# shresthasagar/quantized_spectrum_cartography

Measured on AMD Instinct MI355X. Metric: MLE grad-steps/sec + SLF NMSE, 512x512x256 R=8, higher is better.
Workload: dtype f32; 1 GPU; c3: 512x512 grid, K=256, R=8, one-bit probit, f=0.1, free-S alternating Adam (C-step, S-step); K=256, R=8, parallelism=single, world_size=1, hipgraph=True, nnz_per_gpu=6711192, entry_bytes=2

## Files before the change

### include/qsc.h

```cpp
#ifndef QSC_H_
#define QSC_H_

#include <stddef.h>
#include <stdint.h>

#ifdef __cplusplus
extern "C" {
#endif

#define QSC_API __attribute__((visibility("default")))

#define QSC_OK 0
#define QSC_EINVAL 100000
#define QSC_EUNSUPPORTED 100001
#define QSC_MAX_BOUNDS 256
#define QSC_MAX_R 16
#define QSC_UNOBSERVED 0xFF

typedef struct qsc_model {
  int32_t nbounds;
  int32_t log_model;
  double sigma;
  double offset;
  float bounds[QSC_MAX_BOUNDS];
  int32_t loss;
  int32_t reserved_;
} qsc_model;
#define QSC_LOSS_PROBIT 0
#define QSC_LOSS_SQUARED 1
#define QSC_LOSS_LOGIT 2

typedef struct qsc_adam {
  double lr;
  double beta1;
  double beta2;
  double eps;
  int32_t project_nonneg;
  int32_t pad_;
} qsc_adam;

#define QSC_PEND_C 1
#define QSC_PEND_SNLL 2
#define QSC_PEND_SUPD 4
typedef struct qsc_state {
  int32_t step_c;
  int32_t step_s;
  int32_t iter;
  int32_t pending;
  float normsq_s;
  float normsq_c;
  float nll_c;
  float nll_s;
  float normsq_s_prev;
  int32_t fused_fault;
  uint64_t fin_ticket;
  float reserved[4];
} qsc_state;

#define QSC_SLICE 32
#define QSC_ENTRY_TAIL 256
typedef struct qsc_obs_desc {
  int32_t K;
  int32_t P;
  int32_t Pp;
  int32_t PT;
  int32_t ntiles;
  int32_t nks;
  int32_t wide;
  int32_t nbins;
  int64_t nnz;
  int64_t s_entries;
  int64_t c_entries;
  int32_t rowfmt;
  int32_t reserved_;
} qsc_obs_desc;

QSC_API int qsc_version(void);
QSC_API int qsc_rank_pad(int32_t R);
QSC_API const char* qsc_error_string(int code);
QSC_API int qsc_device_check(int dev);

QSC_API int qsc_quantize(const float* X, const float* noise, int64_t n, const qsc_model* m,
                         int64_t* Y, void* stream);
QSC_API int qsc_bin_codes(const float* x, int64_t n, const qsc_model* m, int64_t* Y,
                          void* stream);
QSC_API int qsc_prob_probit(const int64_t* Y, const float* Xhat, int64_t n, const qsc_model* m,
                            float* P, void* stream);
QSC_API int qsc_prob_probit_bwd(const int64_t* Y, const float* Xhat, const float* gP, int64_t n,
                                const qsc_model* m, float* gX, void* stream);
QSC_API int qsc_f_probit(const float* y, int64_t n, double sigma, float* out, void* stream);
QSC_API int qsc_f_logit(const float* y, int64_t n, double scale, float* out, void* stream);
QSC_API int qsc_prob_logit(const int64_t* Y, const float* Xhat, int64_t n, const qsc_model* m,
                           float* P, void* stream);
QSC_API int qsc_prob_logit_bwd(const int64_t* Y, const float* Xhat, const float* gP, int64_t n,
                               const qsc_model* m, float* gX, void* stream);
QSC_API int qsc_obs_from_ordinal(const int64_t* Y, int64_t n, const qsc_model* m, float* out,
                                 void* stream);
QSC_API int qsc_pack_codes(const int64_t* Y, const float* Wx, int64_t n, int32_t nbins,
                           uint8_t* codes, int32_t* bad, void* stream);

QSC_API int qsc_reconstruct(const float* S, const float* C, int32_t R, int32_t P, int32_t K,
                            float* T, void* stream);
QSC_API size_t qsc_reconstruct_bwd_workspace_bytes(int32_t R, int32_t P, int32_t K);
QSC_API int qsc_reconstruct_bwd(const float* gT, const float* S, const float* C, int32_t R,
                                int32_t P, int32_t K, float* dS, float* dC, void* ws,
                                size_t ws_bytes, void* stream);

QSC_API size_t qsc_reduce_workspace_bytes(int64_t n);
QSC_API int qsc_diff_sumsq(const float* a, const float* b, int64_t n, int32_t use_log,
                           double offset, double* out2, void* ws, size_t ws_bytes, void* stream);
QSC_API int qsc_map_diff_sumsq(const float* S, const float* C, const float* Ttrue, int32_t R,
                               int32_t P, int32_t K, int32_t use_log, double offset,
                               double* out2, void* ws, size_t ws_bytes, void* stream);
QSC_API int qsc_map_nmse_track(const float* S_pos, const int32_t* iperm, int32_t RP,
                               const float* C, const float* Ttrue, int32_t R, int32_t P,
                               int32_t K, int32_t use_log, double offset, const qsc_state* st,
                               int32_t every, double* hist, int32_t cap, void* ws,
                               size_t ws_bytes, void* stream);
QSC_API int qsc_sumsq(const float* x, int64_t n, float* out, void* ws, size_t ws_bytes,
                      void* stream);

QSC_API int qsc_obs_count(const uint8_t* codes, int32_t K, int32_t P, int32_t* cnt, void* stream);
QSC_API size_t qsc_obs_order_workspace_bytes(int32_t P);
QSC_API int qsc_obs_order(const int32_t* cnt, int32_t P, int32_t Pp, int32_t* perm, void* ws,
                          size_t ws_bytes, void* stream);
QSC_API size_t qsc_obs_layout_workspace_bytes(int32_t K, int32_t P, int32_t PT);
QSC_API int qsc_obs_layout(const uint8_t* codes, int32_t K, int32_t P, int32_t PT, int32_t nbins,
                           const int32_t* perm, const int32_t* cnt, int32_t* s_width,
                           int64_t* s_off, int32_t* c_width, int64_t* c_off, int32_t* c_kmap,
                           void* ws, size_t ws_bytes, qsc_obs_desc* desc, void* stream);
QSC_API int qsc_obs_signed_rows_ok(const qsc_obs_desc* desc, int32_t R, const qsc_model* m);
QSC_API int qsc_obs_fill(const uint8_t* codes, const qsc_obs_desc* desc, const int32_t* perm,
                         const int32_t* s_width, const int64_t* s_off, const int32_t* c_width,
                         const int64_t* c_off, const int32_t* c_kmap, void* s_entries,
                         void* c_entries, void* stream);
QSC_API size_t qsc_obs_schedule_workspace_bytes(const qsc_obs_desc* desc);
QSC_API int qsc_obs_schedule(const qsc_obs_desc* desc, const int32_t* s_width,
                             const int64_t* s_off, const int32_t* c_width, const int64_t* c_off,
                             void* s_entries, void* c_entries, void* ws, size_t ws_bytes,
                             void* stream);
QSC_API int qsc_sched_lists_host(const uint32_t* in, uint32_t* out, int32_t W, int32_t rowfmt,
                                 int32_t rows, int32_t wide);
QSC_API int qsc_perm_gather(const float* nat, const int32_t* perm, int32_t R, int32_t P,
                            int32_t Pp, float* pos, void* stream);
QSC_API int qsc_perm_scatter(const float* pos, const int32_t* perm, int32_t R, int32_t P,
                             int32_t Pp, float* nat, void* stream);

QSC_API size_t qsc_pass_workspace_bytes(const qsc_obs_desc* d, int32_t R);
QSC_API int qsc_state_init(qsc_state* st, const float* S, int32_t R, int32_t Pp, void* ws,
                           size_t ws_bytes, void* stream);
QSC_API int qsc_spass(const qsc_obs_desc* d, const void* s_entries, const int32_t* s_width,
                      const int64_t* s_off, const qsc_model* m, int32_t R, float* S,
                      const float* C, int32_t mode, float* dS, float* mS, float* vS,
                      const qsc_adam* adam, float lambda_s, qsc_state* st, void* ws,
                      size_t ws_bytes, void* stream);
QSC_API int qsc_spass_kslab(const qsc_obs_desc* d, const void* s_entries, const int32_t* s_width,
                            const int64_t* s_off, const qsc_model* m, int32_t R, float* S,
                            const float* C, float* dS_rs, int32_t chunk_slices, int32_t nranks,
                            qsc_state* st, void* ws, size_t ws_bytes, void* stream);
QSC_API int qsc_cpass(const qsc_obs_desc* d, const void* c_entries, const int32_t* c_width,
                      const int64_t* c_off, const int32_t* c_kmap, const qsc_model* m, int32_t R,
                      const float* S, const float* C, void* ws, size_t ws_bytes, void* stream);
QSC_API int qsc_scpass_supported(const qsc_obs_desc* d, int32_t R);
QSC_API int qsc_scpass(const qsc_obs_desc* d, const void* s_entries, const int32_t* s_width,
                       const int64_t* s_off, const void* c_entries, const int32_t* c_width,
                       const int64_t* c_off, const int32_t* c_kmap, const qsc_model* m,
                       int32_t R, float* S,
                       const float* C, float* mS, float* vS, const qsc_adam* adam,
                       float lambda_s, qsc_state* st, void* ws, size_t ws_bytes, void* stream);
QSC_API int qsc_cfinish(const qsc_obs_desc* d, int32_t R, float* C, int32_t mode, float* dC,
                        float* mC, float* vC, const qsc_adam* adam, float lambda_c,
                        const float* normsq_c_ext, qsc_state* st, float* hist,
                        int32_t hist_cap, void* ws, size_t ws_bytes, void* stream);
QSC_API int qsc_cupdate(int32_t R, int32_t K, float* C, float* mC, float* vC, const float* g,
                        const qsc_adam* adam, float lambda_c, const float* normsq_s_ext,
                        qsc_state* st, void* stream);
QSC_API int qsc_state_flush(const qsc_obs_desc* d, int32_t R, qsc_state* st, float* hist,
                            int32_t hist_cap, void* ws, size_t ws_bytes, void* stream);
QSC_API int qsc_supdate(const qsc_obs_desc* d, int32_t R, float* S, float* mS, float* vS,
                        const float* g, const qsc_adam* adam, float lambda_s, qsc_state* st,
                        void* ws, size_t ws_bytes, void* stream);
QSC_API int qsc_supdate_slices(const qsc_obs_desc* d, int32_t R, int32_t s0, int32_t s1,
                               float* S, float* mS, float* vS, const float* g_own,
                               const qsc_adam* adam, float lambda_s, qsc_state* st, void* ws,
                               size_t ws_bytes, void* stream);
QSC_API int qsc_slice_nsq(const qsc_obs_desc* d, int32_t R, const float* S, void* ws,
                          size_t ws_bytes, void* stream);
QSC_API int qsc_cpass_nsq(const qsc_obs_desc* d, const void* c_entries, const int32_t* c_width,
                          const int64_t* c_off, const int32_t* c_kmap, const qsc_model* m,
                          int32_t R, const float* S, const float* C, void* ws, size_t ws_bytes,
                          void* stream);
QSC_API int64_t qsc_pass_cnsq_offset(const qsc_obs_desc* d, int32_t R);
QSC_API int qsc_sumsq_small(const float* x, int32_t n, float* out, void* stream);
QSC_API int qsc_adam_flat(float* p, float* m, float* v, const float* g, int64_t n,
                          const qsc_adam* adam, const qsc_state* st, void* stream);
#define QSC_SMOOTH_QUAD 0
#define QSC_SMOOTH_HUBER 1
QSC_API size_t qsc_smooth_workspace_bytes(int32_t Pp);
QSC_API int qsc_smooth_neighbors(const int32_t* perm, int32_t P, int32_t Pp, int32_t I, int32_t J,
                                 int32_t* nbr, void* ws, size_t ws_bytes, void* stream);
QSC_API int qsc_smooth_grad(const float* S, const int32_t* nbr, int32_t R, int32_t Pp,
                            int32_t kind, float delta, float weight, float* dS, float* pen,
                            float* pen_hist, int32_t hist_cap, void* ws, size_t ws_bytes,
                            void* stream);

#define QSC_INFO_EXPECTED 0
#define QSC_INFO_OBSERVED 1
QSC_API int qsc_sinfo(const qsc_obs_desc* d, const void* s_entries, const int32_t* s_width,
                      const int64_t* s_off, const qsc_model* m, int32_t R, const float* S,
                      const float* C, int32_t kind, float* J, void* stream);
QSC_API int qsc_info_std(const float* J, const int32_t* perm, int32_t R, int32_t P, int32_t Pp,
                         const float* C, int32_t K, float ridge, float* std_S, float* std_T,
                         int32_t* nbad, void* stream);
QSC_API int qsc_entry_info(const int64_t* Y, const float* T, int64_t n, const qsc_model* m,
                           int32_t kind, float* H, void* stream);

#define QSC_DESIGN_D 0
#define QSC_DESIGN_A 1
#define QSC_DESIGN_V 2
QSC_API int qsc_sgain(const float* S, const float* C, const float* J, const int32_t* perm,
                      const float* w, const float* G, const qsc_model* m, int32_t R, int32_t K,
                      int32_t P, int32_t Pp, int32_t criterion, float ridge, float* gain,
                      int32_t* n_first, int32_t* n_bad, void* stream);

#define QSC_CHECK_UNTESTABLE 1
#define QSC_CHECK_INVALID 2
#define QSC_CHECK_SATURATED 4
QSC_API int qsc_scheck(const qsc_obs_desc* d, const void* s_entries, const int32_t* s_width,
                       const int64_t* s_off, const int32_t* perm, const qsc_model* m, int32_t R,
                       const float* S, const float* C, int32_t fitted, float ridge, float* stat,
                       int32_t* count, int32_t* flags, void* stream);
QSC_API int qsc_entry_check(const int64_t* Y, const float* T, int64_t n, const qsc_model* m,
                            float* out, void* stream);

QSC_API size_t qsc_sfit_workspace_bytes(const qsc_obs_desc* d, int32_t R);
QSC_API int qsc_sfit(const qsc_obs_desc* d, const void* s_entries, const int32_t* s_width,
                     const int64_t* s_off, const int32_t* perm, const qsc_model* m, int32_t R,
                     const float* C, const float* S_init, int32_t kind, float ridge, float mu0,
                     float tol, int32_t max_steps, int32_t project, float* S_out, float* f_out,
                     int32_t* steps, int32_t* n_unconverged, int32_t* n_unidentified, void* ws,
                     size_t ws_bytes, void* stream);

QSC_API size_t qsc_sfit_smooth_workspace_bytes(const qsc_obs_desc* d, int32_t R);
QSC_API int qsc_sfit_smooth(const qsc_obs_desc* d, const void* s_entries, const int32_t* s_width,
                            const int64_t* s_off, const int32_t* perm, const int32_t* nbr,
                            int32_t I, int32_t J, int32_t color, const qsc_model* m, int32_t R,
                            const float* C, float* S, int32_t kind, float ridge, float mu0,
                            float tol, int32_t inner_steps, int32_t project, int32_t smooth_kind,
                            float delta, float weight, float* f_out, float* nll_out,
                            int32_t* steps, int32_t* n_moved, int32_t* n_unconverged,
                            int32_t* n_unidentified, void* ws, size_t ws_bytes, void* stream);

QSC_API size_t qsc_cfit_workspace_bytes(const qsc_obs_desc* d, int32_t R);
QSC_API int32_t qsc_cfit_groups(const qsc_obs_desc* d, int32_t R);
QSC_API int64_t qsc_cfit_active_offset(void);
QSC_API int qsc_cfit_begin(const qsc_obs_desc* d, const void* c_entries, const int32_t* c_width,
                           const int64_t* c_off, const int32_t* c_kmap, const qsc_model* m,
                           int32_t R, const float* S, const float* C_init, int32_t kind,
                           float ridge, float mu0, float tol, int32_t max_steps, int32_t project,
                           void* ws, size_t ws_bytes, void* stream);
QSC_API int qsc_cfit_iterate(const qsc_obs_desc* d, const void* c_entries, const int32_t* c_width,
                             const int64_t* c_off, const int32_t* c_kmap, const qsc_model* m,
                             int32_t R, const float* S, int32_t kind, void* ws, size_t ws_bytes,
                             void* stream);
QSC_API int qsc_cfit_finish(const qsc_obs_desc* d, const qsc_model* m, int32_t R, float* C_out,
                            double* f_out, int32_t* steps, float* std_C, int32_t* n_unconverged,
                            int32_t* n_unidentified, void* ws, size_t ws_bytes, void* stream);

QSC_API int qsc_debug_status(int32_t clear);
QSC_API int qsc_selftest_erf(const float* x, int32_t n, float* out, void* stream);

QSC_API size_t qsc_gram_workspace_bytes(int32_t R, int32_t P, int32_t K);
QSC_API int qsc_gram(const float* S, const float* w, int32_t R, int32_t P, float* G, void* ws,
                     size_t ws_bytes, void* stream);
QSC_API int qsc_gram_rhs(const float* S, const float* T, const float* w, int32_t R, int32_t P,
                         int32_t K, float* B, void* ws, size_t ws_bytes, void* stream);
QSC_API int qsc_chol_solve(const float* G, const float* B, int32_t R, int32_t K, float lambda,
                           float* X, void* stream);

QSC_API size_t qsc_syrk_workspace_bytes(int32_t K, int32_t P);
QSC_API int qsc_syrk(const float* T, const float* w, int32_t K, int32_t P, float* G, void* ws,
                     size_t ws_bytes, void* stream);
QSC_API size_t qsc_spa_workspace_bytes(int32_t K, int32_t P, int32_t R);
QSC_API int qsc_spa(const float* T, const float* w, int32_t K, int32_t P, int32_t R,
                    int32_t* sel, int32_t* count, float* C, float* S, float* G_out, void* ws,
                    size_t ws_bytes, void* stream);
QSC_API int qsc_nnls(const float* G, const float* B, int32_t R, int32_t K, float lambda,
                     float* X, void* stream);

QSC_API size_t qsc_map_compose_workspace_bytes(int32_t R, int32_t I, int32_t J);
QSC_API int qsc_map_compose(const float* shadow, const float* loc, const float* alpha, int32_t R,
                            int32_t I, int32_t J, float res, float d0, int32_t db, float* S,
                            float* norms, void* ws, size_t ws_bytes, void* stream);

QSC_API int qsc_obs_readings_count(const int32_t* k, const int32_t* p, const void* code,
                                   int32_t code_bytes, int64_t n, int32_t K, int32_t P,
                                   int32_t nbins, int32_t* cnt, int32_t* bad, void* stream);
QSC_API size_t qsc_obs_readings_packed_bytes(int64_t n, int32_t K, int32_t P, int32_t PT);
QSC_API size_t qsc_obs_readings_workspace_bytes(int64_t n, int32_t K, int32_t P, int32_t PT);
QSC_API int qsc_obs_readings_layout(const int32_t* k, const int32_t* p, const void* code,
                                    int32_t code_bytes, int64_t n, int32_t K, int32_t P,
                                    int32_t PT, int32_t nbins, const int32_t* perm,
                                    const int32_t* cnt, int32_t* s_width, int64_t* s_off,
                                    int32_t* c_width, int64_t* c_off, int32_t* c_kmap,
                                    void* packed, size_t packed_bytes, void* ws, size_t ws_bytes,
                                    qsc_obs_desc* desc, int32_t* max_repeat, void* stream);
QSC_API int qsc_obs_readings_fill(const void* packed, size_t packed_bytes, int64_t n,
                                  const qsc_obs_desc* desc, const int32_t* s_width,
                                  const int64_t* s_off, const int32_t* c_width,
                                  const int64_t* c_off, const int32_t* c_kmap, void* s_entries,
                                  void* c_entries, void* stream);

#define QSC_QFIT_SCALE 1
#define QSC_QFIT_SHIFT 2
#define QSC_QFIT_UNCONVERGED 1
#define QSC_QFIT_UNIDENTIFIED 2
QSC_API size_t qsc_qfit_workspace_bytes(const qsc_obs_desc* d, int32_t R);
QSC_API int64_t qsc_qfit_active_offset(void);
QSC_API int qsc_qfit_begin(const qsc_obs_desc* d, const void* s_entries, const int32_t* s_width,
                           const int64_t* s_off, const qsc_model* m, int32_t R, const float* S,
                           const float* C, int32_t kind, int32_t fit_mask, double prior_scale,
                           double prior_shift, double tau0, double beta0, float mu0, float tol,
                           int32_t max_steps, void* ws, size_t ws_bytes, void* stream);
QSC_API int qsc_qfit_iterate(const qsc_obs_desc* d, const void* s_entries, const int32_t* s_width,
                             const int64_t* s_off, const qsc_model* m, int32_t R, const float* S,
                             const float* C, int32_t kind, void* ws, size_t ws_bytes,
                             void* stream);
QSC_API int qsc_qfit_finish(const qsc_obs_desc* d, const qsc_model* m, int32_t R,
                            double* theta_out, double* f_out, double* cov_out, double* gh_out,
                            int32_t* steps, int32_t* flags, void* ws, size_t ws_bytes,
                            void* stream);
QSC_API int qsc_entry_calib(const int64_t* Y, const float* T, int64_t n, const qsc_model* m,
                            double tau, double beta, int32_t kind, double* out, void* stream);

#ifdef __cplusplus
}
#endif
#endif
```

### quantized_spectrum_cartography_amd/csrc/qsc_pass_finish.hip

```cpp
#define QSC_PASS_NO_STAMPS
#include "qsc_pass_host.cuh"

namespace {

struct Canon {
  float nll_s, nsq_s, nll_c;
};

__device__ __forceinline__ float canon_part(const float* __restrict__ x, int n, int tid, int nb) {
  float a = 0.0f;
  if (!x) return a;
  for (int i0 = tid; i0 < n; i0 += 8 * nb) {
    float v[8];
#pragma unroll
    for (int j = 0; j < 8; ++j) v[j] = x[min(i0 + j * nb, n - 1)];
#pragma unroll
    for (int j = 0; j < 8; ++j)
      if (i0 + j * nb < n) a += v[j];
  }
  return a;
}

__device__ Canon canon_totals(const float* __restrict__ nll_s, const float* __restrict__ nsq_s,
                              const float* __restrict__ nll_c, int nslices, int nc, float* sh) {
  const int nb = blockDim.x, tid = threadIdx.x, nw = nb >> 6;
  float a = canon_part(nll_s, nslices, tid, nb);
  float b = canon_part(nsq_s, nslices, tid, nb);
  float c = canon_part(nll_c, nc, tid, nb);
  a = wave_sum(a);
  b = wave_sum(b);
  c = wave_sum(c);
  if ((tid & 63) == 0) {
    sh[tid >> 6] = a;
    sh[nw + (tid >> 6)] = b;
    sh[2 * nw + (tid >> 6)] = c;
  }
  __syncthreads();
  Canon r{0.0f, 0.0f, 0.0f};
  if (tid == 0)
    for (int w = 0; w < nw; ++w) {
      r.nll_s += sh[w];
      r.nsq_s += sh[nw + w];
      r.nll_c += sh[2 * nw + w];
    }
  return r;
}

__device__ void settle_s(qsc_state* __restrict__ st, const float* __restrict__ part_nll_s,
                         const float* __restrict__ part_nsq_s, int nslices, float* hist,
                         int hist_cap, float* sh) {
  const int pend = st->pending;
  if (!(pend & (QSC_PEND_SNLL | QSC_PEND_SUPD))) return;
  const Canon c = canon_totals(part_nll_s, (pend & QSC_PEND_SUPD) ? part_nsq_s : nullptr, nullptr,
                               nslices, 0, sh);
  if (threadIdx.x == 0) {
    const int it = st->iter - 1;
    st->nll_s = c.nll_s;
    if (hist && it >= 0 && it < hist_cap) {
      hist[4 * it + 0] = st->nll_c;
      hist[4 * it + 1] = c.nll_s;
      hist[4 * it + 2] = st->normsq_c;
      hist[4 * it + 3] = st->normsq_s_prev;
    }
    if (pend & QSC_PEND_SUPD) {
      st->normsq_s = c.nsq_s;
      st->step_s += 1;
    }
    st->pending = pend & ~(QSC_PEND_SNLL | QSC_PEND_SUPD);
  }
  __syncthreads();
}

#define QSC_CF_PARAMS                                                                          \
  const float *__restrict__ slab, int ntiles, int nks, int R, int K, float *C, int mode,         \
      float *__restrict__ dC, float *__restrict__ mC, float *__restrict__ vC, qsc_adam ad,       \
      float lambda_c, const float *__restrict__ normsq_ext, const float *__restrict__ cnsq,      \
      qsc_state *__restrict__ st, const float *__restrict__ part_nll_c, int npart_c,             \
      const float *__restrict__ part_nll_s, const float *__restrict__ part_nsq_s, int nslices,   \
      float *__restrict__ hist, int hist_cap, AdamCache *__restrict__ acache
#define QSC_CF_ARGS                                                                           \
  slab, ntiles, nks, R, K, C, mode, dC, mC, vC, ad, lambda_c, normsq_ext, cnsq, st, part_nll_c,  \
      npart_c, part_nll_s, part_nsq_s, nslices, hist, hist_cap, acache
constexpr int kFWaves = kFBlock / 64;

template <int VF>
__device__ __forceinline__ void cfin_tile_sum(float (*red)[64], const float* col,
                                              const int64_t tstride, const int ntiles,
                                              const int wave, const int NWp, const int lane) {
  constexpr int NW = kFWaves, JB = 16 / VF, NGB = 1;
  float a[VF];
#pragma unroll
  for (int f = 0; f < VF; ++f) a[f] = 0.0f;
  for (int tg = 0; tg < ntiles; tg += NGB * 16 * NW) {
    for (int jb = 0; jb < 16; jb += JB) {
      float v[NGB][VF][JB];
#pragma unroll
      for (int gb = 0; gb < NGB; ++gb)
#pragma unroll
        for (int f = 0; f < VF; ++f) {
          const int vw = wave + f * NWp;
#pragma unroll
          for (int j = 0; j < JB; ++j) {
            const int tt = tg + gb * 16 * NW + vw + (jb + j) * NW;
            v[gb][f][j] =
                vw < NW ? col[(int64_t)min(tt, ntiles - 1) * tstride] : 0.0f;
          }
        }
#pragma unroll
      for (int gb = 0; gb < NGB; ++gb)
#pragma unroll
        for (int f = 0; f < VF; ++f) {
          const int vw = wave + f * NWp;
#pragma unroll
          for (int j = 0; j < JB; ++j)
            if (vw < NW && tg + gb * 16 * NW + vw + (jb + j) * NW < ntiles) a[f] += v[gb][f][j];
        }
    }
  }
#pragma unroll
  for (int f = 0; f < VF; ++f)
    if (wave + f * NWp < NW) red[wave + f * NWp][lane] = a[f];
}

__device__ __forceinline__ void cfinish_vb(const int vb, float (*red)[64], Scalars& sc, float* sh,
                                           QSC_CF_PARAMS) {
  constexpr int NW = kFWaves;
  const int NWp = NW;
  const int Kp = nks * 64;
  const int wave = threadIdx.x >> 6, lane = threadIdx.x & 63;

  const float nsq = normsq_ext ? *normsq_ext : *cnsq;

  if (vb == R * nks + 1) {
    if (mode == 1 && threadIdx.x == 0) adam_cache_store(acache, ad, st->step_c + 2);
    return;
  }
  if (vb == R * nks) {
    const int pend = st->pending;
    const bool settle = (pend & (QSC_PEND_SNLL | QSC_PEND_SUPD)) != 0;
    const bool supd = (pend & QSC_PEND_SUPD) != 0;
    const Canon cs = canon_totals(settle ? part_nll_s : nullptr, supd ? part_nsq_s : nullptr,
                                  part_nll_c, nslices, npart_c, sh);
    if (threadIdx.x == 0) {
      int pnd = pend;
      if (settle) {
        const int it = st->iter - 1;
        st->nll_s = cs.nll_s;
        if (hist && it >= 0 && it < hist_cap) {
          hist[4 * it + 0] = st->nll_c;
          hist[4 * it + 1] = cs.nll_s;
          hist[4 * it + 2] = st->normsq_c;
          hist[4 * it + 3] = st->normsq_s_prev;
        }
        if (supd) {
          st->normsq_s = cs.nsq_s;
          st->step_s += 1;
        }
        pnd = pend & ~(QSC_PEND_SNLL | QSC_PEND_SUPD);
        st->pending = pnd;
      }
      st->nll_c = cs.nll_c;
      if (mode == 1) {
        st->normsq_c = nsq;
        st->pending = pnd | QSC_PEND_C;
      }
      if (mode == 2) dC[(int64_t)R * K] = st->normsq_s;
    }
    return;
  }

  const int r = vb / nks, ks = vb - r * nks;
  const int k = ks * 64 + lane;
  float p0 = 0.0f, m0 = 0.0f, v0 = 0.0f;
  if (mode == 1 && wave == 0 && k < K) {
    const int64_t i = (int64_t)r * K + k;
    p0 = C[i];
    m0 = mC[i];
    v0 = vC[i];
  }
  if (threadIdx.x == 0 && mode == 1) {
    const AdamCache a0 = acache[0], a1 = acache[1];
    const int step = st->step_c + 1;
    const float nrm = sqrtf(nsq);
    sc.coef = nrm > 0.0f ? lambda_c / nrm : 0.0f;
    sc.as = adam_scalars_cached((step & 1) ? a1 : a0, ad, step);
  }
  const float* col = slab + (int64_t)r * Kp + k;
  const int64_t tstride = (int64_t)R * Kp;
  cfin_tile_sum<1>(red, col, tstride, ntiles, wave, NWp, lane);
  __syncthreads();
  if (wave == 0 && k < K) {
    float g = red[0][lane];
#pragma unroll
    for (int w = 1; w < NW; ++w) g += red[w][lane];
    const int64_t i = (int64_t)r * K + k;
    if (mode == 1) {
      float p = p0, m = m0, v = v0;
      g = __fadd_rn(g, __fmul_rn(p, sc.coef));
      adam_elem(p, m, v, g, ad, sc.as);
      C[i] = p;
      mC[i] = m;
      vC[i] = v;
    } else {
      dC[i] = g;
    }
  }
}

__global__ void __launch_bounds__(kFBlock) cfinish_kernel(QSC_CF_PARAMS) {
  __shared__ float red[kFWaves][64];
  __shared__ Scalars sc;
  __shared__ float sh[3 * kFWaves];
  cfinish_vb((int)blockIdx.x, red, sc, sh, QSC_CF_ARGS);
}


__global__ void __launch_bounds__(kFBlock) cupdate_kernel(
    int R, int K, float* __restrict__ C, float* __restrict__ mC, float* __restrict__ vC,
    const float* __restrict__ g, qsc_adam ad, float lambda_c,
    const float* __restrict__ normsq_s_ext, qsc_state* __restrict__ st) {
  constexpr int NW = kFBlock / 64;
  __shared__ float shn[NW];
  __shared__ Scalars sc;
  const int n = R * K;
  const float nsq = cnorm_sq(C, n, shn);
  if (threadIdx.x == 0) {
    const float nrm = sqrtf(nsq);
    sc.coef = nrm > 0.0f ? lambda_c / nrm : 0.0f;
    sc.as = adam_scalars(ad, st->step_c + 1);
  }
  __syncthreads();
  for (int i = threadIdx.x; i < n; i += blockDim.x) {
    float p = C[i], m = mC[i], v = vC[i];
    const float gg = __fadd_rn(g[i], __fmul_rn(p, sc.coef));
    adam_elem(p, m, v, gg, ad, sc.as);
    C[i] = p;
    mC[i] = m;
    vC[i] = v;
  }
  if (threadIdx.x == 0) {
    st->normsq_c = nsq;
    st->pending |= QSC_PEND_C;
    if (normsq_s_ext) st->normsq_s = *normsq_s_ext;
  }
}

__global__ void __launch_bounds__(1024) flush_kernel(qsc_state* __restrict__ st,
                                                     const float* __restrict__ part_nll_s,
                                                     const float* __restrict__ part_nsq_s,
                                                     int ntiles, int nslices,
                                                     float* __restrict__ hist, int hist_cap) {
  __shared__ float sh[3 * 16];
  settle_s(st, part_nll_s, part_nsq_s, nslices, hist, hist_cap, sh);
  if (threadIdx.x == 0 && (st->pending & QSC_PEND_C)) {
    st->step_c += 1;
    st->pending &= ~QSC_PEND_C;
  }
}

template <int RP>
__global__ void __launch_bounds__(kSBlock) supdate_kernel(
    int nslices, float* __restrict__ S, float* __restrict__ mS, float* __restrict__ vS,
    const float* __restrict__ gsrc, qsc_adam ad, float lambda_s, qsc_state* __restrict__ st,
    float* __restrict__ part_nsq) {
  constexpr int RH = RP / 2;
  __shared__ Scalars sc;
  if (threadIdx.x == 0) {
    const float nrm = sqrtf(st->normsq_s);
    sc.coef = nrm > 0.0f ? lambda_s / nrm : 0.0f;
    sc.as = adam_scalars(ad, st->step_s + 1);
    if (blockIdx.x == 0) st->pending |= QSC_PEND_SUPD;
  }
  __syncthreads();
  const int wave = threadIdx.x >> 6, lane = threadIdx.x & 63;
  const int s = blockIdx.x * kSWaves + wave;
  if (s >= nslices) return;
  const int64_t o = ((int64_t)s * QSC_SLICE + (lane & (QSC_SLICE - 1))) * RP + (lane >> 5) * RH;
  float p[RH], m[RH], v[RH], g[RH];
  ld_row<RH>(S + o, p);
  ld_row<RH>(mS + o, m);
  ld_row<RH>(vS + o, v);
  ld_row<RH>(gsrc + o, g);
  float nsq = adam_row_fast<RH>(p, m, v, g, sc.coef, sc.as, ad.project_nonneg != 0);
  st_row<RH>(S + o, p);
  st_row<RH>(mS + o, m);
  st_row<RH>(vS + o, v);
  nsq = wave_sum(nsq);
  if (lane == 0) part_nsq[s] = nsq;
}

template <int RP>
__global__ void __launch_bounds__(kSBlock) supdate_slices_kernel(
    int s0, int s1, float* __restrict__ S, float* __restrict__ mS, float* __restrict__ vS,
    const float* __restrict__ g_own, qsc_adam ad, float lambda_s, qsc_state* __restrict__ st,
    float* __restrict__ part_nsq) {
  constexpr int RH = RP / 2;
  __shared__ Scalars sc;
  if (threadIdx.x == 0) {
    const float nrm = sqrtf(st->normsq_s);
    sc.coef = nrm > 0.0f ? lambda_s / nrm : 0.0f;
    sc.as = adam_scalars(ad, st->step_s + 1);
    if (blockIdx.x == 0) st->pending |= QSC_PEND_SUPD;
  }
  __syncthreads();
  const int wave = threadIdx.x >> 6, lane = threadIdx.x & 63;
  const int s = s0 + blockIdx.x * kSWaves + wave;
  if (s >= s1) return;
  const int64_t lo = ((int64_t)(lane & (QSC_SLICE - 1))) * RP + (lane >> 5) * RH;
  const int64_t o = (int64_t)s * QSC_SLICE * RP + lo;
  const int64_t og = (int64_t)(s - s0) * QSC_SLICE * RP + lo;
  float p[RH], m[RH], v[RH], g[RH];
  ld_row<RH>(S + o, p);
  ld_row<RH>(mS + o, m);
  ld_row<RH>(vS + o, v);
  ld_row<RH>(g_own + og, g);
  float nsq = adam_row_fast<RH>(p, m, v, g, sc.coef, sc.as, ad.project_nonneg != 0);
  st_row<RH>(S + o, p);
  st_row<RH>(mS + o, m);
  st_row<RH>(vS + o, v);
  nsq = wave_sum(nsq);
  if (lane == 0) part_nsq[s] = nsq;
}

template <int RP>
__global__ void __launch_bounds__(kSBlock) slice_nsq_kernel(int nslices,
                                                            const float* __restrict__ S,
                                                            float* __restrict__ part_nsq) {
  constexpr int RH = RP / 2;
  const int wave = threadIdx.x >> 6, lane = threadIdx.x & 63;
  const int s = blockIdx.x * kSWaves + wave;
  if (s >= nslices) return;
  const int64_t o = ((int64_t)s * QSC_SLICE + (lane & (QSC_SLICE - 1))) * RP + (lane >> 5) * RH;
  float p[RH];
  ld_row<RH>(S + o, p);
  float nsq = 0.0f;
#pragma unroll
  for (int j = 0; j < RH; ++j) nsq = __builtin_fmaf(p[j], p[j], nsq);
  nsq = wave_sum(nsq);
  if (lane == 0) part_nsq[s] = nsq;
}

__global__ void state_init_kernel(qsc_state* st, const double* nsq_part, int nparts) {
  if (threadIdx.x == 0) {
    double s = 0.0;
    for (int i = 0; i < nparts; ++i) s += nsq_part[i];
    qsc_state z{};
    z.normsq_s = (float)s;
    z.normsq_s_prev = (float)s;
    *st = z;
  }
}

__global__ void __launch_bounds__(kSBlock) nsq_part_kernel(const float* __restrict__ x, int64_t n,
                                                           double* __restrict__ part) {
  __shared__ double sh[kSWaves];
  double s = 0.0;
  for (int64_t i = blockIdx.x * (int64_t)blockDim.x + threadIdx.x; i < n;
       i += (int64_t)gridDim.x * blockDim.x) {
    const double v = x[i];
    s += v * v;
  }
  const double r = block_sum(s, sh);
  if (threadIdx.x == 0) part[blockIdx.x] = r;
}

__global__ void __launch_bounds__(1024) sumsq_small_kernel(const float* __restrict__ x, int n,
                                                           float* __restrict__ out) {
  __shared__ float sh[16];
  const float r = cnorm_sq(x, n, sh);
  if (threadIdx.x == 0) *out = r;
}

__global__ void __launch_bounds__(256) adam_flat_kernel(float* __restrict__ p,
                                                        float* __restrict__ m,
                                                        float* __restrict__ v,
                                                        const float* __restrict__ g, int64_t n,
                                                        qsc_adam ad,
                                                        const qsc_state* __restrict__ st) {
  __shared__ AdamScalars sc;
  if (threadIdx.x == 0) sc = adam_scalars(ad, st->iter);
  __syncthreads();
  const AdamScalars s = sc;
  for (int64_t i = blockIdx.x * (int64_t)blockDim.x + threadIdx.x; i < n;
       i += (int64_t)gridDim.x * blockDim.x) {
    float pp = p[i], mm = m[i], vv = v[i];
    adam_elem(pp, mm, vv, g[i], ad, s);
    p[i] = pp;
    m[i] = mm;
    v[i] = vv;
  }
}

__global__ void selftest_erf_kernel(const float* __restrict__ x, int n, float* __restrict__ out) {
  const int i = blockIdx.x * blockDim.x + threadIdx.x;
  if (i >= n) return;
  out[i] = erff(x[i]);
  out[n + i] = erf_fast(x[i]);
}

}

extern "C" {

QSC_API size_t qsc_pass_workspace_bytes(const qsc_obs_desc* d, int32_t R) {
  if (!desc_ok(d) || R < 1 || R > QSC_MAX_R) return 0;
  return ws_bytes_for(d, R);
}

QSC_API int qsc_state_init(qsc_state* st, const float* S, int32_t R, int32_t Pp, void* ws,
                           size_t ws_bytes, void* stream) {
  if (!st || R < 1 || R > QSC_MAX_R || Pp < 1 || !ws || ws_bytes < 256 * sizeof(double))
    return QSC_EINVAL;
  double* part = (double*)ws;
  const int nb = 256;
  if (S) {
    hipLaunchKernelGGL(nsq_part_kernel, dim3(nb), dim3(kSBlock), 0, STREAM(stream), S,
                       (int64_t)rp_of(R) * Pp, part);
    QSC_CHECK_LAUNCH();
  } else {
    QSC_TRY(hipMemsetAsync(part, 0, nb * sizeof(double), STREAM(stream)));
  }
  hipLaunchKernelGGL(state_init_kernel, dim3(1), dim3(64), 0, STREAM(stream), st, part, nb);
  QSC_CHECK_LAUNCH();
  return QSC_OK;
}

QSC_API int64_t qsc_pass_cnsq_offset(const qsc_obs_desc* d, int32_t R) {
  if (!desc_ok(d) || R < 1 || R > QSC_MAX_R) return -1;
  const uintptr_t base = 4096;
  return (int64_t)(reinterpret_cast<uintptr_t>(carve(d, R, reinterpret_cast<void*>(base)).cnsq) -
                   base);
}

QSC_API int qsc_obs_signed_rows_ok(const qsc_obs_desc* d, int32_t R, const qsc_model* m) {
  if (!desc_ok(d) || !m || R < 1 || R > QSC_MAX_R || m->nbounds - 1 != d->nbins) return 0;
  return (is_onebit_cf(lik_kind(m)) && sr_layout_ok(d, R)) ? 1 : 0;
}

QSC_API int qsc_scpass_supported(const qsc_obs_desc* d, int32_t R) {
  if (!desc_ok(d) || R < 1 || R > 16) return 0;
  return scpass_fits(d, R, d->rowfmt == 1) ? 1 : 0;
}

QSC_API int qsc_cfinish(const qsc_obs_desc* d, int32_t R, float* C, int32_t mode, float* dC,
                        float* mC, float* vC, const qsc_adam* adam, float lambda_c,
                        const float* normsq_c_ext, qsc_state* st, float* hist,
                        int32_t hist_cap, void* ws, size_t ws_bytes, void* stream) {
  if (!desc_ok(d) || R < 1 || R > QSC_MAX_R || !C || !st || !ws || ws_bytes < ws_bytes_for(d, R))
    return QSC_EINVAL;
  if ((mode == 0 || mode == 2) && !dC) return QSC_EINVAL;
  if (mode == 1 && (!mC || !vC || !adam)) return QSC_EINVAL;
  if (mode < 0 || mode > 2) return QSC_EINVAL;
  PassWs w = carve(d, R, ws);
  qsc_adam ad{};
  if (adam) ad = *adam;
  hipLaunchKernelGGL(cfinish_kernel, dim3((unsigned)(R * d->nks + 2)), dim3(kFBlock), 0,
                     STREAM(stream), w.slab, d->ntiles, d->nks, R, d->K, C, mode, dC, mC, vC, ad,
                     lambda_c, normsq_c_ext, w.cnsq, st, w.cnll, d->ntiles * d->nks, w.snll,
                     w.snsq, d->Pp / QSC_SLICE, hist, hist_cap, w.acache + 2);
  QSC_CHECK_LAUNCH();
  return QSC_OK;
}

QSC_API int qsc_cupdate(int32_t R, int32_t K, float* C, float* mC, float* vC, const float* g,
                        const qsc_adam* adam, float lambda_c, const float* normsq_s_ext,
                        qsc_state* st, void* stream) {
  if (R < 1 || R > QSC_MAX_R || K < 1 || !C || !mC || !vC || !g || !adam || !st)
    return QSC_EINVAL;
  hipLaunchKernelGGL(cupdate_kernel, dim3(1), dim3(kFBlock), 0, STREAM(stream), R, K, C, mC, vC,
                     g, *adam, lambda_c, normsq_s_ext, st);
  QSC_CHECK_LAUNCH();
  return QSC_OK;
}

QSC_API int qsc_state_flush(const qsc_obs_desc* d, int32_t R, qsc_state* st, float* hist,
                            int32_t hist_cap, void* ws, size_t ws_bytes, void* stream) {
  if (!desc_ok(d) || R < 1 || R > QSC_MAX_R || !st || !ws || ws_bytes < ws_bytes_for(d, R))
    return QSC_EINVAL;
  PassWs w = carve(d, R, ws);
  hipLaunchKernelGGL(flush_kernel, dim3(1), dim3(1024), 0, STREAM(stream), st, w.snll, w.snsq,
                     d->ntiles, d->Pp / QSC_SLICE, hist, hist_cap);
  QSC_CHECK_LAUNCH();
  return QSC_OK;
}

QSC_API int qsc_supdate(const qsc_obs_desc* d, int32_t R, float* S, float* mS, float* vS,
                        const float* g, const qsc_adam* adam, float lambda_s, qsc_state* st,
                        void* ws, size_t ws_bytes, void* stream) {
  if (!desc_ok(d) || R < 1 || R > QSC_MAX_R || !S || !mS || !vS || !g || !adam || !st || !ws ||
      ws_bytes < ws_bytes_for(d, R))
    return QSC_EINVAL;
  PassWs w = carve(d, R, ws);
  const int nslices = d->Pp / QSC_SLICE;
  const dim3 grid((unsigned)ceil_div(nslices, kSWaves)), blk(kSBlock);
  QSC_LAUNCH_RP(supdate_kernel, rp_of(R), grid, blk, 0, STREAM(stream), nslices, S, mS, vS, g,
                *adam, lambda_s, st, w.snsq);
  QSC_CHECK_LAUNCH();
  return QSC_OK;
}

QSC_API int qsc_supdate_slices(const qsc_obs_desc* d, int32_t R, int32_t s0, int32_t s1,
                               float* S, float* mS, float* vS, const float* g_own,
                               const qsc_adam* adam, float lambda_s, qsc_state* st, void* ws,
                               size_t ws_bytes, void* stream) {
  const int nslices = d ? d->Pp / QSC_SLICE : 0;
  if (!desc_ok(d) || R < 1 || R > QSC_MAX_R || !S || !mS || !vS || !g_own || !adam || !st ||
      !ws || ws_bytes < ws_bytes_for(d, R) || s0 < 0 || s1 < s0 || s1 > nslices)
    return QSC_EINVAL;
  PassWs w = carve(d, R, ws);
  const int n = s1 - s0;
  const dim3 grid((unsigned)std::max<int64_t>(1, ceil_div(n, kSWaves))), blk(kSBlock);
  QSC_LAUNCH_RP(supdate_slices_kernel, rp_of(R), grid, blk, 0, STREAM(stream), s0, s1, S, mS, vS,
                g_own, *adam, lambda_s, st, w.snsq);
  QSC_CHECK_LAUNCH();
  return QSC_OK;
}

QSC_API int qsc_slice_nsq(const qsc_obs_desc* d, int32_t R, const float* S, void* ws,
                          size_t ws_bytes, void* stream) {
  if (!desc_ok(d) || R < 1 || R > QSC_MAX_R || !S || !ws || ws_bytes < ws_bytes_for(d, R))
    return QSC_EINVAL;
  PassWs w = carve(d, R, ws);
  const int nslices = d->Pp / QSC_SLICE;
  const dim3 grid((unsigned)ceil_div(nslices, kSWaves)), blk(kSBlock);
  QSC_LAUNCH_RP(slice_nsq_kernel, rp_of(R), grid, blk, 0, STREAM(stream), nslices, S, w.snsq);
  QSC_CHECK_LAUNCH();
  return QSC_OK;
}

QSC_API int qsc_adam_flat(float* p, float* m, float* v, const float* g, int64_t n,
                          const qsc_adam* adam, const qsc_state* st, void* stream) {
  if (n < 0 || !adam || !st || (n > 0 && (!p || !m || !v || !g))) return QSC_EINVAL;
  if (n == 0) return QSC_OK;
  const int64_t blocks = std::min<int64_t>(ceil_div(n, 256), (int64_t)cu_count() * 8);
  hipLaunchKernelGGL(adam_flat_kernel, dim3((unsigned)blocks), dim3(256), 0, STREAM(stream), p,
                     m, v, g, n, *adam, st);
  QSC_CHECK_LAUNCH();
  return QSC_OK;
}

QSC_API int qsc_sumsq_small(const float* x, int32_t n, float* out, void* stream) {
  if (n < 0 || !x || !out) return QSC_EINVAL;
  hipLaunchKernelGGL(sumsq_small_kernel, dim3(1), dim3(1024), 0, STREAM(stream), x, n, out);
  QSC_CHECK_LAUNCH();
  return QSC_OK;
}

QSC_API int qsc_debug_status(int32_t clear) {
#if QSC_DEBUG
  if (hipDeviceSynchronize() != hipSuccess) return -2;
  const int line[3] = {dbg_line_s(clear != 0), dbg_line_c(clear != 0), dbg_line_fused(clear != 0)};
  for (int f = 0; f < 3; ++f)
    if (line[f] < 0) return -2;
  for (int f = 0; f < 3; ++f)
    if (line[f] > 0) return (f + 1) * 100000 + line[f];
  return 0;
#else
  (void)clear;
  return -1;
#endif
}

QSC_API int qsc_selftest_erf(const float* x, int32_t n, float* out, void* stream) {
  if (n < 0 || !x || !out) return QSC_EINVAL;
  if (n == 0) return QSC_OK;
  hipLaunchKernelGGL(selftest_erf_kernel, dim3((unsigned)ceil_div(n, 256)), dim3(256), 0,
                     STREAM(stream), x, n, out);
  QSC_CHECK_LAUNCH();
  return QSC_OK;
}

}
```

Before: 61910 grad-steps/s.

## Restructure C-finish reduction with fixed 1024-thread blocks and branchless canonical totals

```diff
diff --git a/include/qsc.h b/include/qsc.h
--- a/include/qsc.h
+++ b/include/qsc.h
@@ -191,6 +191,7 @@
                           int32_t R, const float* S, const float* C, void* ws, size_t ws_bytes,
                           void* stream);
 QSC_API int64_t qsc_pass_cnsq_offset(const qsc_obs_desc* d, int32_t R);
+QSC_API int64_t qsc_pass_part_offset(const qsc_obs_desc* d, int32_t R, int32_t which);
 QSC_API int qsc_sumsq_small(const float* x, int32_t n, float* out, void* stream);
 QSC_API int qsc_adam_flat(float* p, float* m, float* v, const float* g, int64_t n,
                           const qsc_adam* adam, const qsc_state* st, void* stream);
diff --git a/quantized_spectrum_cartography_amd/csrc/qsc_pass_finish.hip b/quantized_spectrum_cartography_amd/csrc/qsc_pass_finish.hip
--- a/quantized_spectrum_cartography_amd/csrc/qsc_pass_finish.hip
+++ b/quantized_spectrum_cartography_amd/csrc/qsc_pass_finish.hip
@@ -3,72 +3,93 @@
 
 namespace {
 
+constexpr int kCanon = 1024;
 struct Canon {
   float nll_s, nsq_s, nll_c;
 };
 
-__device__ __forceinline__ float canon_part(const float* __restrict__ x, int n, int tid, int nb) {
-  float a = 0.0f;
-  if (!x) return a;
-  for (int i0 = tid; i0 < n; i0 += 8 * nb) {
-    float v[8];
-#pragma unroll
-    for (int j = 0; j < 8; ++j) v[j] = x[min(i0 + j * nb, n - 1)];
-#pragma unroll
-    for (int j = 0; j < 8; ++j)
-      if (i0 + j * nb < n) a += v[j];
-  }
-  return a;
-}
-
-__device__ Canon canon_totals(const float* __restrict__ nll_s, const float* __restrict__ nsq_s,
-                              const float* __restrict__ nll_c, int nslices, int nc, float* sh) {
-  const int nb = blockDim.x, tid = threadIdx.x, nw = nb >> 6;
-  float a = canon_part(nll_s, nslices, tid, nb);
-  float b = canon_part(nsq_s, nslices, tid, nb);
-  float c = canon_part(nll_c, nc, tid, nb);
-  a = wave_sum(a);
-  b = wave_sum(b);
-  c = wave_sum(c);
-  if ((tid & 63) == 0) {
-    sh[tid >> 6] = a;
-    sh[nw + (tid >> 6)] = b;
-    sh[2 * nw + (tid >> 6)] = c;
+template <int VF, bool WITH_C>
+__device__ __forceinline__ Canon canon_totals(const float* __restrict__ nll_s,
+                                              const float* __restrict__ nsq_s,
+                                              const float* __restrict__ nll_c, int nslices, int nc,
+                                              float* sh) {
+  constexpr int NB = kCanon / VF, NW = kCanon / 64;
+  const int tid = threadIdx.x;
+  float a[VF], b[VF], c[VF];
+#pragma unroll
+  for (int f = 0; f < VF; ++f) a[f] = b[f] = c[f] = 0.0f;
+  const int n = WITH_C ? max(nslices, nc) : nslices;
+  for (int i0 = 0; i0 < n; i0 += 8 * kCanon) {
+    float va[VF][8], vb[VF][8], vc[VF][8];
+#pragma unroll
+    for (int f = 0; f < VF; ++f)
+#pragma unroll
+      for (int j = 0; j < 8; ++j) {
+        const int i = i0 + tid + f * NB + j * kCanon;
+        va[f][j] = nll_s[min(i, nslices - 1)];
+        vb[f][j] = nsq_s[min(i, nslices - 1)];
+        vc[f][j] = WITH_C ? nll_c[min(i, nc - 1)] : 0.0f;
+      }
+#pragma unroll
+    for (int f = 0; f < VF; ++f)
+#pragma unroll
+      for (int j = 0; j < 8; ++j) {
+        const int i = i0 + tid + f * NB + j * kCanon;
+        if (i < nslices) {
+          a[f] += va[f][j];
+          b[f] += vb[f][j];
+        }
+        if (WITH_C && i < nc) c[f] += vc[f][j];
+      }
+  }
+#pragma unroll
+  for (int f = 0; f < VF; ++f) {
+    const float wa = wave_sum(a[f]), wb = wave_sum(b[f]), wc = wave_sum(c[f]);
+    const int w = (tid >> 6) + f * (NB / 64);
+    if ((tid & 63) == 0) {
+      sh[w] = wa;
+      sh[NW + w] = wb;
+      sh[2 * NW + w] = wc;
+    }
   }
   __syncthreads();
   Canon r{0.0f, 0.0f, 0.0f};
   if (tid == 0)
-    for (int w = 0; w < nw; ++w) {
+    for (int w = 0; w < NW; ++w) {
       r.nll_s += sh[w];
-      r.nsq_s += sh[nw + w];
-      r.nll_c += sh[2 * nw + w];
+      r.nsq_s += sh[NW + w];
+      r.nll_c += sh[2 * NW + w];
     }
   return r;
 }
 
-__device__ void settle_s(qsc_state* __restrict__ st, const float* __restrict__ part_nll_s,
-                         const float* __restrict__ part_nsq_s, int nslices, float* hist,
-                         int hist_cap, float* sh) {
-  const int pend = st->pending;
-  if (!(pend & (QSC_PEND_SNLL | QSC_PEND_SUPD))) return;
-  const Canon c = canon_totals(part_nll_s, (pend & QSC_PEND_SUPD) ? part_nsq_s : nullptr, nullptr,
-                               nslices, 0, sh);
-  if (threadIdx.x == 0) {
-    const int it = st->iter - 1;
-    st->nll_s = c.nll_s;
-    if (hist && it >= 0 && it < hist_cap) {
-      hist[4 * it + 0] = st->nll_c;
-      hist[4 * it + 1] = c.nll_s;
-      hist[4 * it + 2] = st->normsq_c;
-      hist[4 * it + 3] = st->normsq_s_prev;
-    }
-    if (pend & QSC_PEND_SUPD) {
-      st->normsq_s = c.nsq_s;
-      st->step_s += 1;
-    }
-    st->pending = pend & ~(QSC_PEND_SNLL | QSC_PEND_SUPD);
-  }
-  __syncthreads();
+struct StateIn {
+  int step_c, step_s, iter, pending;
+  float normsq_s, normsq_c, nll_c, normsq_s_prev;
+};
+__device__ __forceinline__ StateIn state_in(const qsc_state* __restrict__ st) {
+  return StateIn{st->step_c,   st->step_s,   st->iter,  st->pending,
+                 st->normsq_s, st->normsq_c, st->nll_c, st->normsq_s_prev};
+}
+
+__device__ __forceinline__ int settle_store(qsc_state* __restrict__ st, StateIn& s, const Canon& c,
+                                            float* __restrict__ hist, int hist_cap) {
+  const int pend = s.pending;
+  if (!(pend & (QSC_PEND_SNLL | QSC_PEND_SUPD))) return pend;
+  const int it = s.iter - 1;
+  st->nll_s = c.nll_s;
+  if (hist && it >= 0 && it < hist_cap) {
+    hist[4 * it + 0] = s.nll_c;
+    hist[4 * it + 1] = c.nll_s;
+    hist[4 * it + 2] = s.normsq_c;
+    hist[4 * it + 3] = s.normsq_s_prev;
+  }
+  if (pend & QSC_PEND_SUPD) {
+    s.normsq_s = c.nsq_s;
+    st->normsq_s = c.nsq_s;
+    st->step_s = s.step_s + 1;
+  }
+  return pend & ~(QSC_PEND_SNLL | QSC_PEND_SUPD);
 }
 
 #define QSC_CF_PARAMS                                                                          \
@@ -81,104 +102,54 @@
 #define QSC_CF_ARGS                                                                           \
   slab, ntiles, nks, R, K, C, mode, dC, mC, vC, ad, lambda_c, normsq_ext, cnsq, st, part_nll_c,  \
       npart_c, part_nll_s, part_nsq_s, nslices, hist, hist_cap, acache
-constexpr int kFWaves = kFBlock / 64;
-
-template <int VF>
-__device__ __forceinline__ void cfin_tile_sum(float (*red)[64], const float* col,
-                                              const int64_t tstride, const int ntiles,
-                                              const int wave, const int NWp, const int lane) {
-  constexpr int NW = kFWaves, JB = 16 / VF, NGB = 1;
-  float a[VF];
-#pragma unroll
-  for (int f = 0; f < VF; ++f) a[f] = 0.0f;
-  for (int tg = 0; tg < ntiles; tg += NGB * 16 * NW) {
-    for (int jb = 0; jb < 16; jb += JB) {
-      float v[NGB][VF][JB];
-#pragma unroll
-      for (int gb = 0; gb < NGB; ++gb)
-#pragma unroll
-        for (int f = 0; f < VF; ++f) {
-          const int vw = wave + f * NWp;
-#pragma unroll
-          for (int j = 0; j < JB; ++j) {
-            const int tt = tg + gb * 16 * NW + vw + (jb + j) * NW;
-            v[gb][f][j] =
-                vw < NW ? col[(int64_t)min(tt, ntiles - 1) * tstride] : 0.0f;
-          }
-        }
-#pragma unroll
-      for (int gb = 0; gb < NGB; ++gb)
-#pragma unroll
-        for (int f = 0; f < VF; ++f) {
-          const int vw = wave + f * NWp;
-#pragma unroll
-          for (int j = 0; j < JB; ++j)
-            if (vw < NW && tg + gb * 16 * NW + vw + (jb + j) * NW < ntiles) a[f] += v[gb][f][j];
-        }
-    }
-  }
-#pragma unroll
-  for (int f = 0; f < VF; ++f)
-    if (wave + f * NWp < NW) red[wave + f * NWp][lane] = a[f];
-}
-
-__device__ __forceinline__ void cfinish_vb(const int vb, float (*red)[64], Scalars& sc, float* sh,
-                                           QSC_CF_PARAMS) {
-  constexpr int NW = kFWaves;
-  const int NWp = NW;
-  const int Kp = nks * 64;
-  const int wave = threadIdx.x >> 6, lane = threadIdx.x & 63;
+#ifndef QSC_CFIN_GROUP
+#define QSC_CFIN_GROUP 64
+#endif
+constexpr int kFGroup = QSC_CFIN_GROUP, kFParts = 16;
+constexpr int kFinBlock = kFParts * kFGroup;
+static_assert(kFGroup == 16 || kFGroup == 32 || kFGroup == 64, "a 64-bin slice in whole groups");
+
+__global__ void __launch_bounds__(kFinBlock) cfinish_kernel(QSC_CF_PARAMS) {
+  __shared__ float red[kFParts][kFGroup];
+  __shared__ Scalars sc;
+  __shared__ float sh[3 * (kCanon / 64)];
+  const int Kp = nks * 64, ngk = Kp / kFGroup, ncol = R * ngk;
+  const int vb = (int)blockIdx.x, tid = (int)threadIdx.x;
 
   const float nsq = normsq_ext ? *normsq_ext : *cnsq;
 
-  if (vb == R * nks + 1) {
-    if (mode == 1 && threadIdx.x == 0) adam_cache_store(acache, ad, st->step_c + 2);
+  if (vb == ncol + 1) {
+    if (mode == 1 && tid == 0) adam_cache_store(acache, ad, st->step_c + 2);
     return;
   }
-  if (vb == R * nks) {
-    const int pend = st->pending;
-    const bool settle = (pend & (QSC_PEND_SNLL | QSC_PEND_SUPD)) != 0;
-    const bool supd = (pend & QSC_PEND_SUPD) != 0;
-    const Canon cs = canon_totals(settle ? part_nll_s : nullptr, supd ? part_nsq_s : nullptr,
-                                  part_nll_c, nslices, npart_c, sh);
-    if (threadIdx.x == 0) {
-      int pnd = pend;
-      if (settle) {
-        const int it = st->iter - 1;
-        st->nll_s = cs.nll_s;
-        if (hist && it >= 0 && it < hist_cap) {
-          hist[4 * it + 0] = st->nll_c;
-          hist[4 * it + 1] = cs.nll_s;
-          hist[4 * it + 2] = st->normsq_c;
-          hist[4 * it + 3] = st->normsq_s_prev;
-        }
-        if (supd) {
-          st->normsq_s = cs.nsq_s;
-          st->step_s += 1;
-        }
-        pnd = pend & ~(QSC_PEND_SNLL | QSC_PEND_SUPD);
-        st->pending = pnd;
-      }
+  if (vb == ncol) {
+    StateIn s = state_in(st);
+    const Canon cs = canon_totals<kCanon / kFinBlock, true>(part_nll_s, part_nsq_s, part_nll_c,
+                                                            nslices, npart_c, sh);
+    if (tid == 0) {
+      int pnd = settle_store(st, s, cs, hist, hist_cap);
       st->nll_c = cs.nll_c;
       if (mode == 1) {
         st->normsq_c = nsq;
-        st->pending = pnd | QSC_PEND_C;
+        pnd |= QSC_PEND_C;
       }
-      if (mode == 2) dC[(int64_t)R * K] = st->normsq_s;
+      if (pnd != s.pending) st->pending = pnd;
+      if (mode == 2) dC[(int64_t)R * K] = s.normsq_s;
     }
     return;
   }
 
-  const int r = vb / nks, ks = vb - r * nks;
-  const int k = ks * 64 + lane;
+  const int r = vb / ngk, k0 = (vb - r * ngk) * kFGroup;
+  if (k0 >= K) return;
+  const int w = tid / kFGroup, b = tid % kFGroup, k = k0 + b;
+  const int64_t i = (int64_t)r * K + k;
   float p0 = 0.0f, m0 = 0.0f, v0 = 0.0f;
-  if (mode == 1 && wave == 0 && k < K) {
-    const int64_t i = (int64_t)r * K + k;
+  if (mode == 1 && w == 0 && k < K) {
     p0 = C[i];
     m0 = mC[i];
     v0 = vC[i];
   }
-  if (threadIdx.x == 0 && mode == 1) {
+  if (tid == 0 && mode == 1) {
     const AdamCache a0 = acache[0], a1 = acache[1];
     const int step = st->step_c + 1;
     const float nrm = sqrtf(nsq);
@@ -187,13 +158,22 @@
   }
   const float* col = slab + (int64_t)r * Kp + k;
   const int64_t tstride = (int64_t)R * Kp;
-  cfin_tile_sum<1>(red, col, tstride, ntiles, wave, NWp, lane);
+  float a = 0.0f;
+  for (int tg = 0; tg < ntiles; tg += 16 * kFParts) {
+    float v[16];
+#pragma unroll
+    for (int j = 0; j < 16; ++j)
+      v[j] = col[(int64_t)min(tg + w + j * kFParts, ntiles - 1) * tstride];
+#pragma unroll
+    for (int j = 0; j < 16; ++j)
+      if (tg + w + j * kFParts < ntiles) a += v[j];
+  }
+  red[w][b] = a;
   __syncthreads();
-  if (wave == 0 && k < K) {
-    float g = red[0][lane];
-#pragma unroll
-    for (int w = 1; w < NW; ++w) g += red[w][lane];
-    const int64_t i = (int64_t)r * K + k;
+  if (w == 0 && k < K) {
+    float g = red[0][b];
+#pragma unroll
+    for (int q = 1; q < kFParts; ++q) g += red[q][b];
     if (mode == 1) {
       float p = p0, m = m0, v = v0;
       g = __fadd_rn(g, __fmul_rn(p, sc.coef));
@@ -206,14 +186,6 @@
     }
   }
 }
-
-__global__ void __launch_bounds__(kFBlock) cfinish_kernel(QSC_CF_PARAMS) {
-  __shared__ float red[kFWaves][64];
-  __shared__ Scalars sc;
-  __shared__ float sh[3 * kFWaves];
-  cfinish_vb((int)blockIdx.x, red, sc, sh, QSC_CF_ARGS);
-}
-
 
 __global__ void __launch_bounds__(kFBlock) cupdate_kernel(
     int R, int K, float* __restrict__ C, float* __restrict__ mC, float* __restrict__ vC,
@@ -250,11 +222,17 @@
                                                      const float* __restrict__ part_nsq_s,
                                                      int ntiles, int nslices,
                                                      float* __restrict__ hist, int hist_cap) {
-  __shared__ float sh[3 * 16];
-  settle_s(st, part_nll_s, part_nsq_s, nslices, hist, hist_cap, sh);
-  if (threadIdx.x == 0 && (st->pending & QSC_PEND_C)) {
-    st->step_c += 1;
-    st->pending &= ~QSC_PEND_C;
+  __shared__ float sh[3 * (kCanon / 64)];
+  StateIn s = state_in(st);
+  const Canon cs =
+      canon_totals<1, false>(part_nll_s, part_nsq_s, nullptr, nslices, 0, sh);
+  if (threadIdx.x == 0) {
+    int pnd = settle_store(st, s, cs, hist, hist_cap);
+    if (pnd & QSC_PEND_C) {
+      st->step_c = s.step_c + 1;
+      pnd &= ~QSC_PEND_C;
+    }
+    if (pnd != s.pending) st->pending = pnd;
   }
 }
 
@@ -432,6 +410,14 @@
                    base);
 }
 
+QSC_API int64_t qsc_pass_part_offset(const qsc_obs_desc* d, int32_t R, int32_t which) {
+  if (!desc_ok(d) || R < 1 || R > QSC_MAX_R || which < 0 || which > 3) return -1;
+  const uintptr_t base = 4096;
+  const PassWs w = carve(d, R, reinterpret_cast<void*>(base));
+  const float* part[4] = {w.slab, w.cnll, w.snll, w.snsq};
+  return (int64_t)(reinterpret_cast<uintptr_t>(part[which]) - base);
+}
+
 QSC_API int qsc_obs_signed_rows_ok(const qsc_obs_desc* d, int32_t R, const qsc_model* m) {
   if (!desc_ok(d) || !m || R < 1 || R > QSC_MAX_R || m->nbounds - 1 != d->nbins) return 0;
   return (is_onebit_cf(lik_kind(m)) && sr_layout_ok(d, R)) ? 1 : 0;
@@ -454,8 +440,8 @@
   PassWs w = carve(d, R, ws);
   qsc_adam ad{};
   if (adam) ad = *adam;
-  hipLaunchKernelGGL(cfinish_kernel, dim3((unsigned)(R * d->nks + 2)), dim3(kFBlock), 0,
-                     STREAM(stream), w.slab, d->ntiles, d->nks, R, d->K, C, mode, dC, mC, vC, ad,
+  hipLaunchKernelGGL(cfinish_kernel, dim3((unsigned)(R * d->nks * (64 / kFGroup) + 2)),
+                     dim3(kFinBlock), 0, STREAM(stream), w.slab, d->ntiles, d->nks, R, d->K, C, mode, dC, mC, vC, ad,
                      lambda_c, normsq_c_ext, w.cnsq, st, w.cnll, d->ntiles * d->nks, w.snll,
                      w.snsq, d->Pp / QSC_SLICE, hist, hist_cap, w.acache + 2);
   QSC_CHECK_LAUNCH();
```

Result: faster. 62980 grad-steps/s, median of 6 (+1.7%).
